# geoeo/ORB_SLAM3_V1.0

Hardware: AMD Instinct MI355X
Metric: frames/sec ORB extract+match, 752x480 8-level 1000-feat; bit-exact kp/desc (higher is better)
Workload: dtype u8

## Files before the change

orb_slam3_v1.0_amd/csrc/fast_common.h:

```cpp
#pragma once
#include <hip/hip_runtime.h>
#include <stdint.h>

namespace orbfe {

constexpr int kFastTW = 64, kFastTH = 32;

constexpr int kFusedPyramidMinFrames = 0;

__device__ __forceinline__ bool arc9(uint32_t m)
{
    uint32_t m2 = m | (m << 16);
    uint32_t r = m2 & (m2 >> 1);
    r &= r >> 2;
    r &= r >> 4;
    r &= m2 >> 8;
    return (r & 0xffffu) != 0;
}

__device__ __forceinline__ bool corner_at_global(const uint8_t* __restrict__ img, int pitch, int x, int y, int th)
{
    const int8_t dy[16] = {3, 3, 2, 1, 0, -1, -2, -3, -3, -3, -2, -1, 0, 1, 2, 3};
    const int8_t dx[16] = {0, 1, 2, 3, 3, 3, 2, 1, 0, -1, -2, -3, -3, -3, -2, -1};
    const int v = img[(size_t)y * pitch + x];
    uint32_t mb = 0, md = 0;
#pragma unroll
    for (int k = 0; k < 16; k++) {
        const int d = (int)img[(size_t)(y + dy[k]) * pitch + x + dx[k]] - v;
        mb |= (uint32_t)(d > th) << k;
        md |= (uint32_t)(d < -th) << k;
    }
    return arc9(mb) || arc9(md);
}

}
```

orb_slam3_v1.0_amd/csrc/kernels_pyramid.hip:

```cpp
#include <algorithm>
#include <cstdlib>

#include "launch.h"

namespace orbfe {

constexpr int kRsTW = 128, kRsTH = 16;
constexpr int kRsMaxRows = 40, kRsMaxCols = 304;

template <int KPASS>
__global__ __launch_bounds__(256) void resize_kernel(const uint8_t* __restrict__ src, size_t srcFrameStride,
                                                     int sw, int sh, int spitch, int srcAligned4,
                                                     uint8_t* __restrict__ dst, size_t dstFrameStride,
                                                     int dw, int dh, int dpitch,
                                                     const uint32_t* __restrict__ xtab,
                                                     const uint32_t* __restrict__ ytab)
{
    __shared__ __attribute__((aligned(16))) uint8_t sSrc[kRsMaxRows][kRsMaxCols];

    const int f = blockIdx.x;
    const int tx0 = blockIdx.y * kRsTW;
    const int ty0 = blockIdx.z * kRsTH;
    const int tid = threadIdx.x;
    const uint8_t* s = src + (size_t)f * srcFrameStride;

    const int x0 = tx0 + (tid & 31) * 4;
    const int yA = ty0 + (tid >> 5), yB = yA + 8;
    const bool colOk = x0 < dw;
    uint4 xt4 = make_uint4(0, 0, 0, 0);
    uint32_t ytA = 0, ytB = 0;
    if (colOk) xt4 = *reinterpret_cast<const uint4*>(xtab + x0);
    if (yA < dh) ytA = ytab[yA];
    if (yB < dh) ytB = ytab[yB];

    const int txLast = min(tx0 + kRsTW, dw) - 1;
    const int tyLast = min(ty0 + kRsTH, dh) - 1;
    const int sx0 = (int)(xtab[tx0] & 0xffffu) & ~3;
    const int sx1 = min((int)(xtab[txLast] & 0xffffu) + 1, sw - 1);
    const int sy0 = (int)(ytab[ty0] & 0xffffu);
    const int sy1 = min((int)(ytab[tyLast] & 0xffffu) + 1, sh - 1);
    const int nrows = sy1 - sy0 + 1;
    const int ndw = (sx1 - sx0) / 4 + 1;
    const bool staged = nrows <= 4 * KPASS && ndw * 4 <= kRsMaxCols;

    if (staged) {
        const int c4l = tid & 63, rl = tid >> 6;
        if (srcAligned4 && ndw <= 64) {
            constexpr int kPass = KPASS;
            const bool cok = c4l < ndw;
            uint32_t off = __umul24((unsigned)(sy0 + rl), (unsigned)spitch) + (unsigned)(sx0 + 4 * c4l);
            const uint32_t step = 4u * (unsigned)spitch;
            uint32_t wv[kPass];
#pragma unroll
            for (int k = 0; k < kPass; k++) {
// ... 42 lines not shown
                const int x2 = min(x1 + 1, sw - 1);
                const uint32_t a = fetch(y1, x1), b = fetch(y1, x2), c = fetch(y2, x1), e = fetch(y2, x2);
                const uint32_t top = __umul24(a, wxc) + __umul24(b, wx);
                const uint32_t bot = __umul24(c, wxc) + __umul24(e, wx);
                const uint32_t v = __umul24(top, wyc) + __umul24(bot, wy) + (1u << 21);
                outw |= (v >> 22) << (8 * i);
            }
            uint8_t* d = dst + (size_t)f * dstFrameStride + __umul24((unsigned)y, (unsigned)dpitch);
            if (nvalid == 4) {
                *reinterpret_cast<uint32_t*>(d + x0) = outw;
            } else {
                for (int i = 0; i < nvalid; i++) d[x0 + i] = (uint8_t)(outw >> (8 * i));
            }
        }
    };
    if (staged)
        body([&](int yy, int xx) -> uint32_t {
            return (&sSrc[0][0])[__umul24((uint32_t)(yy - sy0), (uint32_t)kRsMaxCols) + (uint32_t)(xx - sx0)];
        });
    else
        body([&](int yy, int xx) -> uint32_t { return s[(size_t)yy * spitch + xx]; });
}


constexpr int kPyrWaves = 4;

constexpr int kPyrRows = 7;
constexpr int kPyrSegDw = 96;
constexpr int kPyrStride = 128;


__device__ __forceinline__ uint32_t mad24_vsv(uint32_t a, uint32_t w, uint32_t c)
{
    uint32_t r;
    asm("v_mad_u32_u24 %0, %1, %2, %3" : "=v"(r) : "v"(a), "s"(w), "v"(c));
    return r;
}

__device__ __forceinline__ void pyr_hpass(uint32_t d0, uint32_t d1, uint32_t d2, const uint32_t (&sel)[4], const uint32_t (&wp)[4],
                                          uint32_t (&h)[4])
{
    typedef unsigned short us2 __attribute__((ext_vector_type(2)));
    const uint32_t e0 = __builtin_amdgcn_alignbyte(d1, d0, 3), e1 = __builtin_amdgcn_alignbyte(d2, d1, 3);
#pragma unroll
    for (int i = 0; i < 4; i++) {
        const uint32_t pair = i < 3 ? __builtin_amdgcn_perm(d1, d0, sel[i]) : __builtin_amdgcn_perm(e1, e0, sel[i]);
        h[i] = __builtin_amdgcn_udot2(__builtin_bit_cast(us2, pair), __builtin_bit_cast(us2, wp[i]), 0u, false);
    }
}

__global__ __launch_bounds__(kPyrWaves * 64) void pyramid_kernel(const PipelineDesc* __restrict__ P, int l, int R,
                                                                 const uint8_t* __restrict__ gray0, size_t gray0FrameStride,
                                                                 int gray0Pitch, uint8_t* __restrict__ ws,
                                                                 const uint32_t* __restrict__ tabs)
{
    __shared__ uint32_t sRows[kPyrWaves][kPyrRows][kPyrStride];

    const int f = blockIdx.x;
    const int lane = threadIdx.x & 63;
    const int wave = __builtin_amdgcn_readfirstlane((int)(threadIdx.x >> 6));
    uint32_t* const ring = &sRows[wave][0][0];

    {
        const LevelDesc& S = P->lv[l - 1];
        const LevelDesc& D = P->lv[l];
        const int sw = S.w, sh = S.h, dw = D.w, dh = D.h, dpitch = D.pitch;
        const uint8_t* src = l == 1 ? gray0 + (size_t)f * gray0FrameStride : ws + S.imgOff + (size_t)f * S.imgFrameStride;
        const int spitch = l == 1 ? gray0Pitch : S.pitch;
        uint8_t* dst = ws + D.imgOff + (size_t)f * D.imgFrameStride;
        const uint32_t* xtab = tabs + D.xtabOff;
        const uint32_t* ytab = tabs + D.ytabOff;
        const int strips = (dh + R - 1) / R, chunks = (dw + 255) / 256;
        const __amdgpu_buffer_rsrc_t srsrc =
            __builtin_amdgcn_make_buffer_rsrc(const_cast<uint8_t*>(src), 0, (sh - 1) * spitch + ((sw + 3) & ~3), 0x00020000);
        const __amdgpu_buffer_rsrc_t drsrc = __builtin_amdgcn_make_buffer_rsrc(dst, 0, dh * dpitch, 0x00020000);

        const int task = (int)blockIdx.y * kPyrWaves + wave;
        if (task < strips * chunks) {
            const int strip = task / chunks, chunk = task - strip * chunks;
            const int x0 = chunk * 256 + lane * 4;
            const bool colOk = x0 < dw;
            const int xg = min(x0, (dw - 1) & ~3);
            const uint4 xt4 = *reinterpret_cast<const uint4*>(xtab + xg);
            const uint32_t xt[4] = {xt4.x, xt4.y, xt4.z, xt4.w};
            const uint32_t start = (xt[0] & 0xffffu) & ~3u;
            const uint32_t segBase = (xtab[chunk * 256] & 0xffffu) & ~3u;
            const uint32_t winOff = start - segBase;
            uint32_t sel[4], wp[4];
#pragma unroll
            for (int i = 0; i < 4; i++) {
                const uint32_t o = (xt[i] & 0xffffu) - start - (i == 3 ? 3u : 0u);
                sel[i] = 0x0c000c00u | o | ((o + 1u) << 16);
                const uint32_t wx = xt[i] >> 16;
                wp[i] = (2048u - wx) | (wx << 16);
            }
            const int nvalid = min(4, dw - x0);
            constexpr uint32_t kNowhere = 0x7ffffff0u;
            const uint32_t rowEnd = (uint32_t)((sw + 3) & ~3);
            const uint32_t colA = segBase + 4u * (uint32_t)lane;
            const uint32_t ldA = colA + 4u <= rowEnd ? colA : kNowhere;
            const uint32_t ldB = (lane < kPyrSegDw - 64 && colA + 260u <= rowEnd) ? colA + 256u : kNowhere;
            const uint32_t stX = colOk ? (uint32_t)x0 : kNowhere;
            const bool partial = (dw & 3) != 0;

            const int ys = strip * R, ye = min(ys + R, dh);
            const uint32_t roMax = (uint32_t)((sh - 1) * spitch);
            uint32_t kRound = 1u << 23;
            asm("" : "+v"(kRound));
            uint32_t ytN[4];
            uint32_t ga[kPyrRows], gb[kPyrRows];
            auto request = [&](int yb) {
// ... 48 lines not shown
                                    __builtin_amdgcn_raw_buffer_store_b8((uint8_t)(outw >> (8 * i)), drsrc, (uint32_t)(x0 + i), stRow, 0);
                            }
                        }
                    }
                    stRow += (uint32_t)dpitch;
                }
            }
        }
    }
}

void launch_resize(hipStream_t s, int frames, const uint8_t* src, size_t srcFrameStride, int sw, int sh,
                   int spitch, int srcAligned4, uint8_t* dst, size_t dstFrameStride, int dw, int dh, int dpitch,
                   const uint32_t* xtab, const uint32_t* ytab)
{
    dim3 block(256);
    dim3 grid(frames, (dw + kRsTW - 1) / kRsTW, (dh + kRsTH - 1) / kRsTH);
    const int maxRows = (int)(((long long)(kRsTH - 1) * sh + dh - 1) / dh) + 2;
    if (maxRows <= 24)
        hipLaunchKernelGGL(resize_kernel<6>, grid, block, 0, s, src, srcFrameStride, sw, sh, spitch, srcAligned4, dst,
                           dstFrameStride, dw, dh, dpitch, xtab, ytab);
    else
        hipLaunchKernelGGL(resize_kernel<kRsMaxRows / 4>, grid, block, 0, s, src, srcFrameStride, sw, sh, spitch, srcAligned4,
                           dst, dstFrameStride, dw, dh, dpitch, xtab, ytab);
}


bool pyramid_level_fits(const uint32_t* xtab, const uint32_t* ytab, int sw, int sh, int dw, int dh)
{
    for (int y = 0; y < dh; y++) {
        if ((int)(ytab[y] & 0xffffu) + 1 > sh - 1) return false;
        const int yl = std::min(y + 3, dh - 1);
        if ((int)(ytab[yl] & 0xffffu) + 1 - (int)(ytab[y] & 0xffffu) + 1 > kPyrRows) return false;
    }
    for (int c0 = 0; c0 < dw; c0 += 256) {
        const uint32_t segBase = (xtab[c0] & 0xffffu) & ~3u;
        const int xl = (std::min(c0 + 256, dw) - 1) & ~3;
        const uint32_t startL = (xtab[xl] & 0xffffu) & ~3u;
        if (startL + 12 - segBase > 4u * kPyrSegDw) return false;
    }
    for (int x0 = 0; x0 < dw; x0 += 4) {
        const uint32_t start = (xtab[x0] & 0xffffu) & ~3u;
        for (int i = 0; i < 4 && x0 + i < dw; i++) {
            const uint32_t x1 = xtab[x0 + i] & 0xffffu;
            if ((int)x1 + 1 > sw - 1 || x1 < start) return false;
            const uint32_t o = x1 - start;
            if (i < 3 ? o + 1 > 7 : (o < 3 || o - 3 + 1 > 7)) return false;
        }
    }
    return true;
}

void launch_pyramid_level(hipStream_t s, int frames, const PipelineDesc* dP, int level, int dw, int dh, const uint8_t* gray0,
                          size_t gray0FrameStride, int gray0Pitch, uint8_t* ws, const uint32_t* tabs)
{
#ifdef ORBFE_DIAG
    static const int envR = getenv("ORBFE_PYR_ROWS") ? atoi(getenv("ORBFE_PYR_ROWS")) : 0;
#else
    constexpr int envR = 0;
#endif
    const int R = envR > 0 ? (envR + 3) & ~3 : frames >= 128 ? 8 : 4;
    const int tasks = ((dh + R - 1) / R) * ((dw + 255) / 256);
    hipLaunchKernelGGL(pyramid_kernel, dim3(frames, (tasks + kPyrWaves - 1) / kPyrWaves), dim3(kPyrWaves * 64), 0, s, dP, level, R, gray0,
                       gray0FrameStride, gray0Pitch, ws, tabs);
}


namespace {

struct ChainCtx {
    const uint8_t* src0;
    int pitch0, w0, h0;
    const uint32_t* xtab[3];
    const uint32_t* ytab[3];
    int w[3], h[3];
};

template <int K>
__device__ __forceinline__ uint32_t chain_px(const ChainCtx& c, int x, int y)
{
    const uint32_t xt = c.xtab[K - 1][x], yt = c.ytab[K - 1][y];
    const int sw = K == 1 ? c.w0 : c.w[K - 2], sh = K == 1 ? c.h0 : c.h[K - 2];
    const int x1 = (int)(xt & 0xffffu), y1 = (int)(yt & 0xffffu);
    const uint32_t wx = xt >> 16, wy = yt >> 16;
    const uint32_t wxc = 2048u - wx, wyc = 2048u - wy;
    const int x2 = min(x1 + 1, sw - 1), y2 = min(y1 + 1, sh - 1);
    uint32_t a, b, cc, e;
    if constexpr (K == 1) {
        const uint8_t* r1 = c.src0 + (size_t)y1 * c.pitch0;
        const uint8_t* r2 = c.src0 + (size_t)y2 * c.pitch0;
        a = r1[x1]; b = r1[x2]; cc = r2[x1]; e = r2[x2];
    } else {
        a = chain_px<K - 1>(c, x1, y1); b = chain_px<K - 1>(c, x2, y1);
        cc = chain_px<K - 1>(c, x1, y2); e = chain_px<K - 1>(c, x2, y2);
    }
    const uint32_t top = __umul24(a, wxc) + __umul24(b, wx);
    const uint32_t bot = __umul24(cc, wxc) + __umul24(e, wx);
    const uint32_t v = __umul24(top, wyc) + __umul24(bot, wy) + (1u << 21);
    return v >> 22;
}

__global__ __launch_bounds__(256) void pyramid_chain_kernel(const PipelineDesc* __restrict__ P, int l0, int depth,
                                                            const uint8_t* __restrict__ gray0, size_t gray0FrameStride, int gray0Pitch,
                                                            uint8_t* __restrict__ ws, const uint32_t* __restrict__ tabs,
                                                            uint32_t* __restrict__ zero, int nZeroPerFrame)
{
    const int f = blockIdx.y;
    if (zero && blockIdx.x == 0)
        for (int i = threadIdx.x; i < nZeroPerFrame; i += 256) zero[(size_t)f * nZeroPerFrame + i] = 0;
    ChainCtx c;
    const LevelDesc& S = P->lv[l0];
    c.src0 = l0 == 0 ? gray0 + (size_t)f * gray0FrameStride : ws + S.imgOff + (size_t)f * S.imgFrameStride;
    c.pitch0 = l0 == 0 ? gray0Pitch : S.pitch;
    c.w0 = S.w;
    c.h0 = S.h;
    int np[3] = {0, 0, 0};
#pragma unroll
    for (int k = 0; k < 3; k++) {
// ... 36 lines not shown
```

orb_slam3_v1.0_amd/csrc/launch.h:

```cpp
#pragma once
#include "orbfe_internal.h"

namespace orbfe {

void launch_resize(hipStream_t s, int frames, const uint8_t* src, size_t srcFrameStride, int sw, int sh,
                   int spitch, int srcAligned4, uint8_t* dst, size_t dstFrameStride, int dw, int dh, int dpitch,
                   const uint32_t* xtab, const uint32_t* ytab);

bool pyramid_level_fits(const uint32_t* xtab, const uint32_t* ytab, int sw, int sh, int dw, int dh);
void launch_pyramid_level(hipStream_t s, int frames, const PipelineDesc* dP, int level, int dw, int dh, const uint8_t* gray0,
                          size_t gray0FrameStride, int gray0Pitch, uint8_t* ws, const uint32_t* tabs);

void launch_pyramid_chain(hipStream_t s, int frames, const PipelineDesc* dP, const PipelineDesc& hostP, int l0, int depth,
                          const uint8_t* gray0, size_t gray0FrameStride, int gray0Pitch, uint8_t* ws, const uint32_t* tabs,
                          uint32_t* zero = nullptr, int nZeroPerFrame = 0);

void fast_tiles_for(int w, int h, int* tx, int* ty);
uint32_t fast_tile_info(int level, int tileX, int tileY);
void launch_fast_blur(hipStream_t s, int frames, int tileBase, int nTiles, bool buildNext, const PipelineDesc* dP,
                      const uint32_t* dTileInfo, const uint32_t* dTabs, const uint8_t* gray0, size_t gray0FrameStride, int gray0Pitch,
                      int gray0Aligned4, uint8_t* ws, uint32_t* cand, uint32_t* counters, uint16_t* tileRows);
bool fast_next_level_fits(const uint32_t* xtab, const uint32_t* ytab, int sw, int sh, int dw, int dh, uint32_t* own);

int quadtree_node_capacity(int maxNodeCap);
size_t quadtree_scratch_bytes_per_block(int maxNodeCap);
void launch_quadtree(hipStream_t s, int frames, int nLevels, int maxNodeCap, const PipelineDesc* dP,
                     const uint32_t* cand, uint16_t* nodeOf, uint32_t* counters, uint32_t* lvlKp,
                     const uint8_t* gray0, size_t gray0FrameStride, int gray0Pitch, const uint8_t* ws,
                     const uint16_t* tileRows, uint8_t* scratch);

void launch_orient_brief(hipStream_t s, int frames, int kpCapFrame, const PipelineDesc* dP, const uint8_t* gray0,
                         size_t gray0FrameStride, int gray0Pitch, const uint8_t* ws, const uint32_t* counters,
                         const uint32_t* lvlKp, orbfe_keypoint* kpOut, uint8_t* descOut, int* nOut,
                         int* perLevelOut, int* statusOut, const int* kpBase, int nLevels);

void launch_clock_probe(hipStream_t s, unsigned long long* dOut2, unsigned ticks);

}
```

orb_slam3_v1.0_amd/csrc/orbfe_host.cpp:

```cpp
#include <atomic>
#include <cmath>
#include <cstdio>
#include <cstdlib>
#include <cstring>
#include <map>
#include <mutex>
#include <new>
#include <condition_variable>
#include <functional>
#include <string>
#include <thread>
#include <vector>

#include "launch.h"
#include "fast_common.h"
#include "match.h"
#include "match_common.h"
#include "match_proj.h"
#include "keyframe.h"
#include "marginalize.h"
#include "poseimu_math.h"
#include "prep.h"
#include "vocab.h"

// ... 18 lines not shown
        Key key;
        hipGraphExec_t exec;
    };
    std::vector<Entry> entries;
    hipGraphExec_t find(const Key& key) const
    {
        for (const Entry& e : entries)
            if (memcmp(&e.key, &key, sizeof key) == 0) return e.exec;
        return nullptr;
    }
    void insert(const Key& key, hipGraphExec_t exec, size_t bound)
    {
        if (entries.size() >= bound) drop();
        entries.push_back({key, exec});
    }
    void drop()
    {
        for (Entry& e : entries)
            if (e.exec) (void)hipGraphExecDestroy(e.exec);
        entries.clear();
    }
};

}

struct orbfe_map;
struct orbfe_stream;

struct orbfe_handle {
    orbfe_params prm{};
    int device = 0;
    int nLevels = 0;
    double scaleFactorD = 0.0;
    float sf[kMaxLevels]{}, inv[kMaxLevels]{}, sig2[kMaxLevels]{}, invSig2[kMaxLevels]{};
    PipelineDesc P{};
    PipelineDesc* dP = nullptr;
    int maxBatch = 1;
    int maxNodeCap = 0;

    uint8_t* ws = nullptr;
    size_t wsBytes = 0;
    uint32_t* dCand = nullptr;
    uint16_t* dNodeOf = nullptr;
    size_t candWordsPerBatch = 0;
    uint32_t* dCounters = nullptr;
    uint32_t* dLvlKp = nullptr;
    uint16_t* dTileRows = nullptr;
    uint8_t* dQtScratch = nullptr;
    uint32_t* dTabs = nullptr;
    uint32_t* dTileInfo = nullptr;
    bool pyrFits[kMaxLevels]{};
    bool fusedFits[kMaxLevels]{};
    int fusedMinFrames = kFusedPyramidMinFrames;
    bool fusedSplitOnly = false;
    float* dSf = nullptr;

    uint8_t* dIn = nullptr;
    int dInPitch = 0;
    uint8_t* hIn = nullptr;
    uint8_t* dOutBlock = nullptr;
    uint8_t* hOutBlock = nullptr;
    size_t outBlockBytes = 0, offStatus = 0, offPer = 0, offKp = 0, offDesc = 0;
    orbfe_keypoint* dKp = nullptr;
    uint8_t* dDesc = nullptr;
    int* dN = nullptr;
    int* dStatus = nullptr;
    int* dPer = nullptr;
    orbfe_keypoint* hKp = nullptr;
    uint8_t* hDesc = nullptr;
    int* hN = nullptr;
    int* hStatus = nullptr;
    int* hPer = nullptr;
    std::map<int, hipGraphExec_t> graphs;
    bool useGraph = true;
    int graphCaptures = 0, captureFailures = 0;
    int captureFailStreak = 0;

    hipStream_t stream = nullptr;
    bool timing = false;
    hipEvent_t ev[kEventSets][ORBFE_NUM_STAGES]{};
    int evHead = 0, evCount = 0;

    const uint8_t* lastGray = nullptr;
    size_t lastStride = 0;
    int lastPitch = 0, lastBatch = 0;

    MatchScratch match;

    struct TrackKey {
        int Mb, inPitch, gridCols, gridRows, farPoints;
        float minX, minY, invW, invH, th, nnRatio, thFar;
        const void* map;
    };
    MatchScratch trackMatch;
    ChainBlocks trk;
    int trkCapM = 0;
    GraphCache<TrackKey> trackGraphs;
    struct RefKey {
        int inPitch, levelsup, checkOri;
        float nnRatio;
        unsigned long long vocabSerial;
    };
    ChainBlocks ref;
    int refCapFlags = 0;
    GraphCache<RefKey> refGraphs;
    struct IniKey {
// ... 243 lines not shown
    PipelineDesc& P = h->P;
    memset(&P, 0, sizeof P);
    P.nLevels = nL;
    P.nFast = p->n_fast_features;
    P.iniTh = p->ini_th_fast;
    P.minTh = p->min_th_fast;
    size_t wsOff = 0, candOff = 0, tabOff = 0;
    int tileBase = 0, kpBase = 0;
    const size_t B = (size_t)p->max_batch;
    int status = ORBFE_OK;
    for (int l = 0; l < nL; l++) {
        LevelDesc& L = P.lv[l];
        if (l == 0) {
            L.w = p->image_width;
            L.h = p->image_height;
        } else {
            L.w = cv_round_f(h->inv[l] * (float)p->image_width);
            L.h = cv_round_f(h->inv[l] * (float)p->image_height);
        }
        if (L.w < 16 || L.h < 16) { status = ORBFE_ERR_UNSUPPORTED; break; }
        L.pitch = (int)align_up((size_t)L.w, kPitchAlign);
        L.nFeatures = fpl[l];
        L.nIni = (int)roundf((float)L.w / (float)L.h);
        if (L.nIni < 1) { status = ORBFE_ERR_UNSUPPORTED; break; }
        L.hX = (float)L.w / (float)L.nIni;
        L.nodeCap = std::max(L.nFeatures + 3, 4 * L.nIni);
        L.candCap = ((L.w + 1) / 2) * ((L.h + 1) / 2);
        fast_tiles_for(L.w, L.h, &L.tilesX, &L.tilesY);
        L.tileBase = tileBase;
        tileBase += L.tilesX * L.tilesY;
        L.kpBase = kpBase;
        kpBase += L.nodeCap;
        L.invScale = h->inv[l];
        L.scaledPatch = (int)(kPatch * h->inv[l]);
        const size_t frameBytes = align_up((size_t)L.pitch * L.h, 256);
        L.imgFrameStride = frameBytes;
        L.blurFrameStride = frameBytes;
        if (l > 0) {
            L.imgOff = wsOff;
            wsOff += frameBytes * B;
        }
        L.blurOff = wsOff;
        wsOff += frameBytes * B;
        L.candOff = candOff;
        candOff += (size_t)L.candCap * B;
        tabOff = align_up(tabOff, 4);
        L.xtabOff = tabOff;
        tabOff += align_up((size_t)L.w, 4);
        L.ytabOff = tabOff;
        tabOff += align_up((size_t)L.h, 4);
        tabOff = align_up(tabOff, 4);
        L.ownOff = (uint32_t)tabOff;
        tabOff += (size_t)L.tilesX + L.tilesY + 2;
        h->maxNodeCap = std::max(h->maxNodeCap, L.nodeCap);
    }
    if (status == ORBFE_OK && quadtree_node_capacity(h->maxNodeCap) == 0) status = ORBFE_ERR_UNSUPPORTED;
    if (status != ORBFE_OK) {
        delete h;
        return status;
    }
    P.kpCapFrame = kpBase;
    P.totalTiles = tileBase;
    for (int l = 0; l < 8; l++) P.tileBaseTab[l] = l < nL ? P.lv[l].tileBase : 0x7fffffff;
    h->wsBytes = wsOff;
    h->candWordsPerBatch = candOff;

    std::vector<uint32_t> tabs(tabOff ? tabOff : 1, 0);
    for (int l = 1; l < nL; l++) {
        fill_resize_table(tabs, P.lv[l].xtabOff, P.lv[l - 1].w, P.lv[l].w);
        fill_resize_table(tabs, P.lv[l].ytabOff, P.lv[l - 1].h, P.lv[l].h);
    }

    for (int l = 1; l < nL; l++)
        if (pyramid_level_fits(tabs.data() + P.lv[l].xtabOff, tabs.data() + P.lv[l].ytabOff, P.lv[l - 1].w, P.lv[l - 1].h, P.lv[l].w,
                               P.lv[l].h))
            h->pyrFits[l] = true;
    for (int l = 1; l < nL; l++)
        h->fusedFits[l] = fast_next_level_fits(tabs.data() + P.lv[l].xtabOff, tabs.data() + P.lv[l].ytabOff, P.lv[l - 1].w, P.lv[l - 1].h,
                                               P.lv[l].w, P.lv[l].h, tabs.data() + P.lv[l - 1].ownOff) && h->pyrFits[l];

#define CREATE_CHK(call)                                                  \
    do {                                                                  \
        hipError_t e_ = (call);                                           \
        if (e_ != hipSuccess) {                                           \
            int rc_ = e_ == hipErrorOutOfMemory ? ORBFE_ERR_OUT_OF_MEMORY : ORBFE_ERR_HIP; \
            destroy_impl(h);                                              \
            return rc_;                                                   \
        }                                                                 \
    } while (0)

    CREATE_CHK(hipStreamCreateWithFlags(&h->stream, hipStreamNonBlocking));
    CREATE_CHK(hipMalloc(&h->dP, sizeof(PipelineDesc)));
    CREATE_CHK(hipMalloc(&h->ws, h->wsBytes + 256));
    CREATE_CHK(hipMalloc(&h->dCand, candOff * sizeof(uint32_t)));
    CREATE_CHK(hipMalloc(&h->dNodeOf, candOff * sizeof(uint16_t)));
    CREATE_CHK(hipMalloc(&h->dCounters, B * nL * kCntWords * sizeof(uint32_t)));
    CREATE_CHK(hipMalloc(&h->dLvlKp, B * (size_t)P.kpCapFrame * sizeof(uint32_t)));
    CREATE_CHK(hipMalloc(&h->dTileRows, B * (size_t)P.totalTiles * 32 * sizeof(uint16_t)));
    if (quadtree_scratch_bytes_per_block(h->maxNodeCap))
        CREATE_CHK(hipMalloc(&h->dQtScratch, quadtree_scratch_bytes_per_block(h->maxNodeCap) * B * nL));
    CREATE_CHK(hipMalloc(&h->dTabs, tabs.size() * sizeof(uint32_t)));
    {
        std::vector<uint32_t> info((size_t)P.totalTiles);
        for (int l = 0; l < nL; l++)
            for (int ty = 0; ty < P.lv[l].tilesY; ty++)
                for (int tx = 0; tx < P.lv[l].tilesX; tx++) info[P.lv[l].tileBase + ty * P.lv[l].tilesX + tx] = fast_tile_info(l, tx, ty);
        CREATE_CHK(hipMalloc(&h->dTileInfo, info.size() * sizeof(uint32_t)));
        CREATE_CHK(copy_sync(h->dTileInfo, info.data(), info.size() * sizeof(uint32_t), hipMemcpyHostToDevice, h->stream));
    }
    CREATE_CHK(hipMalloc(&h->dSf, kMaxLevels * sizeof(float)));
    CREATE_CHK(copy_sync(h->dSf, h->sf, kMaxLevels * sizeof(float), hipMemcpyHostToDevice, h->stream));
    CREATE_CHK(copy_sync(h->dP, &P, sizeof P, hipMemcpyHostToDevice, h->stream));
    CREATE_CHK(copy_sync(h->dTabs, tabs.data(), tabs.size() * sizeof(uint32_t), hipMemcpyHostToDevice, h->stream));

    h->dInPitch = (int)align_up((size_t)p->image_width, kPitchAlign);
    const size_t inFrame = (size_t)h->dInPitch * p->image_height;
    const size_t cap = (size_t)P.kpCapFrame;
    CREATE_CHK(hipMalloc(&h->dIn, inFrame * B));
    CREATE_CHK(hipHostMalloc(&h->hIn, inFrame * B));
    {
        size_t off = 0;
        auto take = [&](size_t bytes) { const size_t o = off; off = align_up(off + bytes, 256); return o; };
        take(B * sizeof(int));
        h->offStatus = take(B * sizeof(int));
        h->offPer = take(B * nL * sizeof(int));
        h->offKp = take(B * cap * sizeof(orbfe_keypoint));
        h->offDesc = take(B * cap * ORBFE_DESC_BYTES);
        h->outBlockBytes = off;
    }
    CREATE_CHK(hipMalloc(&h->dOutBlock, h->outBlockBytes));
    CREATE_CHK(hipHostMalloc(&h->hOutBlock, h->outBlockBytes));
    h->dN = reinterpret_cast<int*>(h->dOutBlock);
    h->dStatus = reinterpret_cast<int*>(h->dOutBlock + h->offStatus);
    h->dPer = reinterpret_cast<int*>(h->dOutBlock + h->offPer);
    h->dKp = reinterpret_cast<orbfe_keypoint*>(h->dOutBlock + h->offKp);
    h->dDesc = h->dOutBlock + h->offDesc;
    h->hN = reinterpret_cast<int*>(h->hOutBlock);
    h->hStatus = reinterpret_cast<int*>(h->hOutBlock + h->offStatus);
    h->hPer = reinterpret_cast<int*>(h->hOutBlock + h->offPer);
    h->hKp = reinterpret_cast<orbfe_keypoint*>(h->hOutBlock + h->offKp);
    h->hDesc = h->hOutBlock + h->offDesc;
#ifdef ORBFE_DIAG
    h->useGraph = getenv("ORBFE_NO_GRAPH") == nullptr;
    if (const char* e = getenv("ORBFE_FUSED_PYRAMID")) {
        h->fusedMinFrames = atoi(e) ? 1 : 0;
        h->fusedSplitOnly = atoi(e) == 2;
    }
#endif
    CREATE_CHK(hipEventCreateWithFlags(&h->evExtract, hipEventDisableTiming));
    CREATE_CHK(hipEventCreateWithFlags(&h->evMatch, hipEventDisableTiming));
    h->match.busy = h->evMatch;
    for (auto& set : h->ev)
        for (auto& e : set) CREATE_CHK(hipEventCreate(&e));
#undef CREATE_CHK
    *out = h;
    return ORBFE_OK;
}

void orbfe_destroy(orbfe_handle* h) { destroy_impl(h); }

int orbfe_get_levels(const orbfe_handle* h) { return h ? h->nLevels : 0; }
float orbfe_get_scale_factor(const orbfe_handle* h) { return h ? (float)h->scaleFactorD : 0.f; }

int orbfe_get_scale_tables(const orbfe_handle* h, float* sf, float* inv, float* s2, float* is2)
{
    if (!h) return ORBFE_ERR_INVALID_ARG;
    for (int i = 0; i < h->nLevels; i++) {
        if (sf) sf[i] = h->sf[i];
        if (inv) inv[i] = h->inv[i];
        if (s2) s2[i] = h->sig2[i];
        if (is2) is2[i] = h->invSig2[i];
    }
    return ORBFE_OK;
}

int orbfe_get_level_info(const orbfe_handle* h, int* fpl, int* lw, int* lh)
{
    if (!h) return ORBFE_ERR_INVALID_ARG;
    for (int i = 0; i < h->nLevels; i++) {
        if (fpl) fpl[i] = h->P.lv[i].nFeatures;
        if (lw) lw[i] = h->P.lv[i].w;
        if (lh) lh[i] = h->P.lv[i].h;
    }
    return ORBFE_OK;
}

int orbfe_max_keypoints(const orbfe_handle* h) { return h ? h->P.kpCapFrame : 0; }

int orbfe_set_stage_timing(orbfe_handle* h, int enabled)
{
    if (!h) return ORBFE_ERR_INVALID_ARG;
    h->timing = enabled != 0;
    h->evHead = h->evCount = 0;
    return ORBFE_OK;
}

int orbfe_get_stage_ms(orbfe_handle* h, float ms[ORBFE_NUM_STAGES], int* n_calls)
{
    if (!h || !ms || !n_calls) return ORBFE_ERR_INVALID_ARG;
    HIPCHK(h, hipSetDevice(h->device));
// ... 7 lines not shown
            HIPCHK(h, hipEventElapsedTime(&t, e[s], e[s + 1]));
            ms[s] += t;
        }
        float t = 0.f;
        HIPCHK(h, hipEventElapsedTime(&t, e[0], e[ORBFE_NUM_STAGES - 1]));
        ms[ORBFE_NUM_STAGES - 1] += t;
    }
    *n_calls = n;
    return ORBFE_OK;
}

static int extract_chain(orbfe_handle* h, const uint8_t* d_gray, size_t frame_stride, int pitch, int batch,
                         orbfe_keypoint* d_kp, uint8_t* d_desc, int* d_n, int* d_per, int* d_status, void* stream_);

int orbfe_extract_batch_device(orbfe_handle* h, const uint8_t* d_gray, size_t frame_stride, int pitch,
                               int batch, orbfe_keypoint* d_kp, uint8_t* d_desc, int* d_n, int* d_per,
                               void* stream_)
{
    if (!h) return ORBFE_ERR_INVALID_ARG;
    std::lock_guard<std::mutex> lk(h->mu);
    return extract_chain(h, d_gray, frame_stride, pitch, batch, d_kp, d_desc, d_n, d_per, nullptr, stream_);
}

}

static int extract_chain(orbfe_handle* h, const uint8_t* d_gray, size_t frame_stride, int pitch, int batch,
                         orbfe_keypoint* d_kp, uint8_t* d_desc, int* d_n, int* d_per, int* d_status, void* stream_)
{
    if (!h || !d_gray || !d_kp || !d_desc || !d_n) return ORBFE_ERR_INVALID_ARG;
    if (batch < 1 || batch > h->maxBatch || pitch < h->prm.image_width || pitch >= (1 << 24)) return ORBFE_ERR_INVALID_ARG;
    const int aligned4 = ((reinterpret_cast<uintptr_t>(d_gray) | (uintptr_t)pitch | (uintptr_t)frame_stride) & 3u) == 0;
    const size_t rowEnd = aligned4 ? (size_t)((h->prm.image_width + 3) & ~3) : (size_t)h->prm.image_width;
    if (batch > 1 && frame_stride < (size_t)pitch * (h->prm.image_height - 1) + rowEnd) return ORBFE_ERR_INVALID_ARG;
    if ((size_t)pitch * (h->prm.image_height - 1) + (size_t)((h->prm.image_width + 3) & ~3) >= (size_t)0x7ffffff0u)
        return ORBFE_ERR_INVALID_ARG;
    HIPCHK(h, hipSetDevice(h->device));
    hipStream_t s = stream_ ? (hipStream_t)stream_ : h->stream;
    hipStreamCaptureStatus capturing = hipStreamCaptureStatusNone;
    if (hipStreamIsCapturing(s, &capturing) != hipSuccess) (void)hipGetLastError();
    if (capturing == hipStreamCaptureStatusNone) {
        const int rc = scratch_acquire(h, h->extractUsed, h->extractStream, h->evExtract, s);
        if (rc != ORBFE_OK) return rc;
    }
    const PipelineDesc& P = h->P;
    const int nL = P.nLevels;
    hipEvent_t* ev = nullptr;
    if (h->timing) {
        ev = h->ev[h->evHead];
        h->evHead = (h->evHead + 1) % kEventSets;
        h->evCount++;
    }
    const bool fused = h->fusedMinFrames > 0 && batch >= h->fusedMinFrames && nL > 1;
    const bool chainPyr = !fused && (long long)batch * nL <= 64 && !ev && nL > 1;
    if (!chainPyr) HIPCHK(h, hipMemsetAsync(h->dCounters, 0, (size_t)batch * nL * kCntWords * sizeof(uint32_t), s));
    if (ev) HIPCHK(h, hipEventRecord(ev[0], s));
    for (int l = 1; chainPyr && l < nL;) {
        const int left = nL - l;
        const int depth = left >= 5 ? 2 : std::min(left, 3);
        launch_pyramid_chain(s, batch, h->dP, P, l - 1, depth, d_gray, frame_stride, pitch, h->ws, h->dTabs,
                             l == 1 ? h->dCounters : nullptr, nL * kCntWords);
        l += depth;
    }
    auto pyramid_level = [&](int l) {
        const LevelDesc& S = P.lv[l - 1];
        const LevelDesc& D = P.lv[l];
        if (h->pyrFits[l] && (l > 1 || aligned4)) {
            launch_pyramid_level(s, batch, h->dP, l, D.w, D.h, d_gray, frame_stride, pitch, h->ws, h->dTabs);
            return;
        }
        const uint8_t* src = l == 1 ? d_gray : h->ws + S.imgOff;
        const size_t sstride = l == 1 ? frame_stride : S.imgFrameStride;
        const int spitch = l == 1 ? pitch : S.pitch;
        launch_resize(s, batch, src, sstride, S.w, S.h, spitch, l == 1 ? aligned4 : 1, h->ws + D.imgOff, D.imgFrameStride, D.w, D.h,
                      D.pitch, h->dTabs + D.xtabOff, h->dTabs + D.ytabOff);
    };
    for (int l = chainPyr || (fused && !h->fusedSplitOnly) ? nL : 1; l < nL; l++) pyramid_level(l);
    if (ev) HIPCHK(h, hipEventRecord(ev[1], s));
    if (fused) {
        for (int l = 0; l < nL; l++) {
            const bool build = l + 1 < nL && h->fusedFits[l + 1] && !h->fusedSplitOnly;
            launch_fast_blur(s, batch, P.lv[l].tileBase, P.lv[l].tilesX * P.lv[l].tilesY, build, h->dP, h->dTileInfo, h->dTabs, d_gray,
                             frame_stride, pitch, aligned4, h->ws, h->dCand, h->dCounters, h->dTileRows);
            if (l + 1 < nL && !build && !h->fusedSplitOnly) pyramid_level(l + 1);
        }
    } else {
        launch_fast_blur(s, batch, 0, P.totalTiles, false, h->dP, h->dTileInfo, h->dTabs, d_gray, frame_stride, pitch, aligned4, h->ws,
                         h->dCand, h->dCounters, h->dTileRows);
    }
    if (ev) HIPCHK(h, hipEventRecord(ev[2], s));
    launch_quadtree(s, batch, nL, h->maxNodeCap, h->dP, h->dCand, h->dNodeOf, h->dCounters, h->dLvlKp, d_gray, frame_stride,
                    pitch, h->ws, h->dTileRows, h->dQtScratch);
    if (ev) HIPCHK(h, hipEventRecord(ev[3], s));
    int kpBase[kMaxLevels];
    for (int l = 0; l < nL; l++) kpBase[l] = P.lv[l].kpBase;
    launch_orient_brief(s, batch, P.kpCapFrame, h->dP, d_gray, frame_stride, pitch, h->ws, h->dCounters, h->dLvlKp,
                        d_kp, d_desc, d_n, d_per, d_status, kpBase, nL);
    if (ev) HIPCHK(h, hipEventRecord(ev[4], s));
    HIPCHK(h, hipGetLastError());
    h->lastGray = d_gray;
    h->lastStride = frame_stride;
    h->lastPitch = pitch;
    h->lastBatch = batch;
    if (capturing == hipStreamCaptureStatusNone) return extract_scratch_release(h, s);
    return ORBFE_OK;
}

extern "C" {

static int check_device_flags(orbfe_handle* h, int batch)
{
    for (int b = 0; b < batch; b++)
        if (h->hStatus[b]) {
            char buf[128];
            snprintf(buf, sizeof buf, "device guard flags 0x%x at frame %d", (unsigned)h->hStatus[b], b);
            h->err = buf;
            return ORBFE_ERR_INTERNAL;
        }
    return ORBFE_OK;
}

static int extract_host_enqueue(orbfe_handle* h, int batch, int inPitch, hipStream_t s)
{
    const int nL = h->nLevels;
    const size_t inFrame = (size_t)h->dInPitch * h->prm.image_height;
    const size_t cap = (size_t)h->P.kpCapFrame;
    const int rc = extract_chain(h, h->dIn, inFrame, inPitch, batch, h->dKp, h->dDesc, h->dN, h->dPer, h->dStatus, s);
    if (rc != ORBFE_OK) return rc;
    if (batch == h->maxBatch) {
        HIPCHK(h, hipMemcpyAsync(h->hOutBlock, h->dOutBlock, h->outBlockBytes, hipMemcpyDeviceToHost, s));
// ... 2657 lines not shown
```

Measured before the change: 228,200.

## Add paired pyramid kernel and fold counter clearing into first pyramid launch

Adds a kernel that builds two consecutive pyramid levels in one pass. Each wave keeps the intermediate level rows in an LDS ring buffer and resizes them again for the next level, which saves one launch and one global re-read per pair. A host-side check works out column and row ownership tables so every intermediate row is stored exactly once. Separately, the counter hipMemsetAsync is replaced by zeroing done inside the first pyramid launch. The pair path is gated by kPyramidPairMinFrames, which is 0, so by default it stays off unless ORBFE_PYR_PAIR is set in diag builds. The memset folding does run by default on the non-chain, non-fused path.

```diff
diff --git a/orb_slam3_v1.0_amd/csrc/fast_common.h b/orb_slam3_v1.0_amd/csrc/fast_common.h
--- a/orb_slam3_v1.0_amd/csrc/fast_common.h
+++ b/orb_slam3_v1.0_amd/csrc/fast_common.h
@@ -7,6 +7,8 @@
 constexpr int kFastTW = 64, kFastTH = 32;
 
 constexpr int kFusedPyramidMinFrames = 0;
+
+constexpr int kPyramidPairMinFrames = 0;
 
 __device__ __forceinline__ bool arc9(uint32_t m)
 {
diff --git a/orb_slam3_v1.0_amd/csrc/kernels_pyramid.hip b/orb_slam3_v1.0_amd/csrc/kernels_pyramid.hip
--- a/orb_slam3_v1.0_amd/csrc/kernels_pyramid.hip
+++ b/orb_slam3_v1.0_amd/csrc/kernels_pyramid.hip
@@ -1,5 +1,6 @@
 #include <algorithm>
 #include <cstdlib>
+#include <vector>
 
 #include "launch.h"
 
@@ -148,11 +149,14 @@
 __global__ __launch_bounds__(kPyrWaves * 64) void pyramid_kernel(const PipelineDesc* __restrict__ P, int l, int R,
                                                                  const uint8_t* __restrict__ gray0, size_t gray0FrameStride,
                                                                  int gray0Pitch, uint8_t* __restrict__ ws,
-                                                                 const uint32_t* __restrict__ tabs)
+                                                                 const uint32_t* __restrict__ tabs, uint32_t* __restrict__ zero,
+                                                                 int nZeroPerFrame)
 {
     __shared__ uint32_t sRows[kPyrWaves][kPyrRows][kPyrStride];
 
     const int f = blockIdx.x;
+    if (zero && blockIdx.y == 0)
+        for (int i = threadIdx.x; i < nZeroPerFrame; i += kPyrWaves * 64) zero[(size_t)f * nZeroPerFrame + i] = 0;
     const int lane = threadIdx.x & 63;
     const int wave = __builtin_amdgcn_readfirstlane((int)(threadIdx.x >> 6));
     uint32_t* const ring = &sRows[wave][0][0];
@@ -307,7 +311,7 @@
 }
 
 void launch_pyramid_level(hipStream_t s, int frames, const PipelineDesc* dP, int level, int dw, int dh, const uint8_t* gray0,
-                          size_t gray0FrameStride, int gray0Pitch, uint8_t* ws, const uint32_t* tabs)
+                          size_t gray0FrameStride, int gray0Pitch, uint8_t* ws, const uint32_t* tabs, uint32_t* zero, int nZeroPerFrame)
 {
 #ifdef ORBFE_DIAG
     static const int envR = getenv("ORBFE_PYR_ROWS") ? atoi(getenv("ORBFE_PYR_ROWS")) : 0;
@@ -317,8 +321,279 @@
     const int R = envR > 0 ? (envR + 3) & ~3 : frames >= 128 ? 8 : 4;
     const int tasks = ((dh + R - 1) / R) * ((dw + 255) / 256);
     hipLaunchKernelGGL(pyramid_kernel, dim3(frames, (tasks + kPyrWaves - 1) / kPyrWaves), dim3(kPyrWaves * 64), 0, s, dP, level, R, gray0,
-                       gray0FrameStride, gray0Pitch, ws, tabs);
-}
+                       gray0FrameStride, gray0Pitch, ws, tabs, zero, nZeroPerFrame);
+}
+
+
+constexpr int kPairWaves = 3;
+constexpr int kPairRows = 16;
+constexpr int kPairRing = 8;
+constexpr int kPairMinCw = 64;
+constexpr int kPairWaveDw = kPairRing * 64 + kPyrRows * kPyrSegDw;
+
+__global__ __launch_bounds__(kPairWaves * 64) void pyramid_pair_kernel(const PipelineDesc* __restrict__ P, int l, int cw, uint32_t pairTab,
+                                                                      const uint8_t* __restrict__ gray0, size_t gray0FrameStride,
+                                                                      int gray0Pitch, uint8_t* __restrict__ ws,
+                                                                      const uint32_t* __restrict__ tabs, uint32_t* __restrict__ zero,
+                                                                      int nZeroPerFrame)
+{
+    __shared__ uint32_t sMem[kPairWaves][kPairWaveDw];
+
+    const int f = blockIdx.x;
+    if (zero && blockIdx.y == 0)
+        for (int i = threadIdx.x; i < nZeroPerFrame; i += kPairWaves * 64) zero[(size_t)f * nZeroPerFrame + i] = 0;
+    const int lane = threadIdx.x & 63;
+    const int wave = __builtin_amdgcn_readfirstlane((int)(threadIdx.x >> 6));
+    uint32_t* const ring = &sMem[wave][0];
+    uint32_t* const stage = ring + kPairRing * 64;
+
+    const LevelDesc& A = P->lv[l - 1];
+    const LevelDesc& B = P->lv[l];
+    const LevelDesc& C = P->lv[l + 1];
+    const int wA = A.w, hA = A.h, wB = B.w, hB = B.h, pitchB = B.pitch, wC = C.w, hC = C.h, pitchC = C.pitch;
+    const uint8_t* src = l == 1 ? gray0 + (size_t)f * gray0FrameStride : ws + A.imgOff + (size_t)f * A.imgFrameStride;
+    const int spitch = l == 1 ? gray0Pitch : A.pitch;
+    uint8_t* dstB = ws + B.imgOff + (size_t)f * B.imgFrameStride;
+    uint8_t* dstC = ws + C.imgOff + (size_t)f * C.imgFrameStride;
+    const uint32_t* xtB = tabs + B.xtabOff;
+    const uint32_t* ytB = tabs + B.ytabOff;
+    const uint32_t* xtC = tabs + C.xtabOff;
+    const uint32_t* ytC = tabs + C.ytabOff;
+    const int strips = (hC + kPairRows - 1) / kPairRows, chunks = (wC + cw - 1) / cw;
+    const uint32_t* colOwn = tabs + pairTab;
+    const uint32_t* rowOwn = colOwn + chunks + 1;
+    const __amdgpu_buffer_rsrc_t srsrc =
+        __builtin_amdgcn_make_buffer_rsrc(const_cast<uint8_t*>(src), 0, (hA - 1) * spitch + ((wA + 3) & ~3), 0x00020000);
+    const __amdgpu_buffer_rsrc_t rsrcB = __builtin_amdgcn_make_buffer_rsrc(dstB, 0, hB * pitchB, 0x00020000);
+    const __amdgpu_buffer_rsrc_t rsrcC = __builtin_amdgcn_make_buffer_rsrc(dstC, 0, hC * pitchC, 0x00020000);
+
+    const int task = (int)blockIdx.y * kPairWaves + wave;
+    if (task >= strips * chunks) return;
+    const int strip = task / chunks, chunk = task - strip * chunks;
+    const int bLo = (int)colOwn[chunk], ownHiX = (int)colOwn[chunk + 1];
+    const int ownLoY = (int)rowOwn[strip], ownHiY = (int)rowOwn[strip + 1];
+    constexpr uint32_t kNowhere = 0x7ffffff0u;
+
+    const int xB0 = bLo + lane * 4;
+    uint32_t selB[4], wpB[4], winOffA;
+    const uint32_t segBase = (xtB[bLo] & 0xffffu) & ~3u;
+    {
+        const uint4 xt4 = *reinterpret_cast<const uint4*>(xtB + min(xB0, (wB - 1) & ~3));
+        const uint32_t xt[4] = {xt4.x, xt4.y, xt4.z, xt4.w};
+        const uint32_t start = (xt[0] & 0xffffu) & ~3u;
+        winOffA = min(start - segBase, 4u * (kPyrSegDw - 3));
+#pragma unroll
+        for (int i = 0; i < 4; i++) {
+            const uint32_t o = (xt[i] & 0xffffu) - start - (i == 3 ? 3u : 0u);
+            selB[i] = 0x0c000c00u | o | ((o + 1u) << 16);
+            const uint32_t wx = xt[i] >> 16;
+            wpB[i] = (2048u - wx) | (wx << 16);
+        }
+    }
+    const bool ownB = xB0 < ownHiX;
+    const int nvalidB = min(4, wB - xB0);
+    const uint32_t stXB = ownB ? (uint32_t)xB0 : kNowhere;
+    const bool partialB = (wB & 3) != 0;
+    const uint32_t rowEnd = (uint32_t)((wA + 3) & ~3);
+    const uint32_t colA = segBase + 4u * (uint32_t)lane;
+    const uint32_t ldA = colA + 4u <= rowEnd ? colA : kNowhere;
+    const uint32_t ldB = (lane < kPyrSegDw - 64 && colA + 260u <= rowEnd) ? colA + 256u : kNowhere;
+
+    const int xC0 = chunk * cw + lane * 4;
+    const bool colOkC = lane * 4 < cw && xC0 < wC;
+    uint32_t selC[4], wpC[4], winOffC;
+    {
+        const uint4 xt4 = *reinterpret_cast<const uint4*>(xtC + min(xC0, (wC - 1) & ~3));
+        const uint32_t xt[4] = {xt4.x, xt4.y, xt4.z, xt4.w};
+        const uint32_t start = (xt[0] & 0xffffu) & ~3u;
+        winOffC = min(start - (uint32_t)bLo, 252u);
+#pragma unroll
+        for (int i = 0; i < 4; i++) {
+            const uint32_t o = (xt[i] & 0xffffu) - start - (i == 3 ? 3u : 0u);
+            selC[i] = 0x0c000c00u | o | ((o + 1u) << 16);
+            const uint32_t wx = xt[i] >> 16;
+            wpC[i] = (2048u - wx) | (wx << 16);
+        }
+    }
+    const int nvalidC = min(4, wC - xC0);
+    const uint32_t stXC = colOkC ? (uint32_t)xC0 : kNowhere;
+    const bool partialC = (wC & 3) != 0;
+
+    const int ys = strip * kPairRows, ye = min(ys + kPairRows, hC);
+    const int bStart = ownLoY;
+    const int bEnd = strip == strips - 1 ? hB : (int)(ytC[ye - 1] & 0xffffu) + 2;
+    const uint32_t roMax = (uint32_t)((hA - 1) * spitch);
+    uint32_t kRound = 1u << 23;
+    asm("" : "+v"(kRound));
+
+    auto blend = [&](const uint32_t* wt, const uint32_t* wb, const uint32_t (&sel)[4], const uint32_t (&wp)[4], uint32_t ytEntry) {
+        uint32_t hT[4], hU[4];
+        pyr_hpass(wt[0], wt[1], wt[2], sel, wp, hT);
+        pyr_hpass(wb[0], wb[1], wb[2], sel, wp, hU);
+        const uint32_t wy4 = (ytEntry >> 16) * 4u, wyc4 = 8192u - wy4;
+        uint32_t v[4];
+#pragma unroll
+        for (int i = 0; i < 4; i++) v[i] = mad24_vsv(hU[i], wy4, mad24_vsv(hT[i], wyc4, kRound));
+        const uint32_t lo = __builtin_amdgcn_perm(v[1], v[0], 0x0c0c0703u);
+        const uint32_t hi = __builtin_amdgcn_perm(v[3], v[2], 0x0c0c0703u);
+        return lo | (hi << 16);
+    };
+    auto put = [&](uint32_t outw, const __amdgpu_buffer_rsrc_t& rsrc, bool partial, bool colOk, int nvalid, int x0, uint32_t stX,
+                   uint32_t stRow) {
+        if (!partial) {
+            __builtin_amdgcn_raw_buffer_store_b32(outw, rsrc, stX, stRow, 0);
+        } else if (colOk) {
+            if (nvalid >= 4) {
+                __builtin_amdgcn_raw_buffer_store_b32(outw, rsrc, (uint32_t)x0, stRow, 0);
+            } else {
+                for (int i = 0; i < nvalid; i++)
+                    __builtin_amdgcn_raw_buffer_store_b8((uint8_t)(outw >> (8 * i)), rsrc, (uint32_t)(x0 + i), stRow, 0);
+            }
+        }
+    };
+
+    uint32_t ytN[4];
+    uint32_t ga[kPyrRows], gb[kPyrRows];
+    auto request = [&](int b) {
+#pragma unroll
+        for (int k = 0; k < 4; k++) ytN[k] = ytB[min(b + k, hB - 1)];
+        uint32_t ro = (ytN[0] & 0xffffu) * (uint32_t)spitch;
+#pragma unroll
+        for (int j = 0; j < kPyrRows; j++) {
+            const uint32_t roc = min(ro, roMax);
+            ga[j] = __builtin_amdgcn_raw_buffer_load_b32(srsrc, ldA, roc, 0);
+            gb[j] = __builtin_amdgcn_raw_buffer_load_b32(srsrc, ldB, roc, 0);
+            ro += (uint32_t)spitch;
+        }
+    };
+    request(bStart);
+    int yC = ys;
+    uint32_t ytC4[4];
+#pragma unroll
+    for (int k = 0; k < 4; k++) ytC4[k] = ytC[min(yC + k, hC - 1)];
+    uint32_t stRowC = (uint32_t)(ys * pitchC);
+    uint32_t stRowB = (uint32_t)(bStart * pitchB);
+#pragma unroll 1
+    for (int b = bStart; b < bEnd; b += 4) {
+        uint32_t yt[4];
+#pragma unroll
+        for (int k = 0; k < 4; k++) yt[k] = ytN[k];
+        const int rA = (int)(yt[0] & 0xffffu);
+#pragma unroll
+        for (int j = 0; j < kPyrRows; j++) stage[j * kPyrSegDw + lane] = ga[j];
+        if (lane < kPyrSegDw - 64) {
+#pragma unroll
+            for (int j = 0; j < kPyrRows; j++) stage[j * kPyrSegDw + 64 + lane] = gb[j];
+        }
+        if (b + 4 < bEnd) request(b + 4);
+#pragma unroll
+        for (int k = 0; k < 4; k++) {
+            if (b + k >= bEnd) break;
+            const int jt = (int)(yt[k] & 0xffffu) - rA;
+            const uint32_t* wt = reinterpret_cast<const uint32_t*>(reinterpret_cast<const uint8_t*>(stage + jt * kPyrSegDw) + winOffA);
+            const uint32_t outw = blend(wt, wt + kPyrSegDw, selB, wpB, yt[k]);
+            ring[((b + k) & (kPairRing - 1)) * 64 + lane] = outw;
+            if (b + k < ownHiY) put(outw, rsrcB, partialB, ownB, nvalidB, xB0, stXB, stRowB);
+            stRowB += (uint32_t)pitchB;
+        }
+        const int bDone = b + 4;
+        uint32_t ytU[4];
+        bool go[4];
+        int n = 0;
+#pragma unroll
+        for (int k = 0; k < 4; k++) {
+            ytU[k] = ytC4[k];
+            go[k] = yC + k < ye && (int)(ytU[k] & 0xffffu) + 1 < bDone;
+            n += go[k] ? 1 : 0;
+        }
+        yC += n;
+#pragma unroll
+        for (int k = 0; k < 4; k++) ytC4[k] = ytC[min(yC + k, hC - 1)];
+#pragma unroll
+        for (int k = 0; k < 4; k++) {
+            if (go[k]) {
+                const int y1 = (int)(ytU[k] & 0xffffu);
+                const uint32_t* wt = reinterpret_cast<const uint32_t*>(
+                    reinterpret_cast<const uint8_t*>(ring + (y1 & (kPairRing - 1)) * 64) + winOffC);
+                const uint32_t* wb = reinterpret_cast<const uint32_t*>(
+                    reinterpret_cast<const uint8_t*>(ring + ((y1 + 1) & (kPairRing - 1)) * 64) + winOffC);
+                const uint32_t outw = blend(wt, wb, selC, wpC, ytU[k]);
+                put(outw, rsrcC, partialC, colOkC, nvalidC, xC0, stXC, stRowC);
+                stRowC += (uint32_t)pitchC;
+            }
+        }
+    }
+}
+
+int pyramid_pair_fits(const uint32_t* xtB, const uint32_t* ytB, const uint32_t* xtC, const uint32_t* ytC, int wB, int hB, int wC, int hC,
+                      uint32_t* own, int ownCap)
+{
+    auto near = [](const uint32_t* t, int i) { return (int)(t[i] & 0xffffu); };
+    const int strips = (hC + kPairRows - 1) / kPairRows;
+    int cw = 0, chunks = 0;
+    const int nMin = (wC + 255) / 256;
+    for (int n = nMin; cw == 0; n++) {
+        const int w = ((wC + n - 1) / n + 3) & ~3;
+        if (n > nMin && w < kPairMinCw) return 0;
+        const int nc = (wC + w - 1) / w;
+        if (nc + 1 + strips + 1 > ownCap) return 0;
+        bool ok = true;
+        for (int c = 0; c <= nc; c++) own[c] = c == nc ? (uint32_t)wB : (uint32_t)(near(xtC, c * w) & ~3);
+        for (int c = 0; c < nc && ok; c++) {
+            const int bLo = (int)own[c], hi = (int)own[c + 1];
+            const int xLast = std::min((c + 1) * w, wC) - 1;
+            const int need = std::max(hi - 1, near(xtC, xLast) + 1);
+            ok = hi > bLo && bLo < wB && need < wB && need - bLo < 256;
+            for (int x0 = c * w; x0 <= xLast && ok; x0 += 4) ok = (near(xtC, x0) & ~3) - bLo <= 252;
+            if (ok) ok = (near(xtB, need & ~3) & ~3) + 12 - (near(xtB, bLo) & ~3) <= 4 * kPyrSegDw;
+        }
+        if (ok) { cw = w; chunks = nc; }
+    }
+    uint32_t* rowOwn = own + chunks + 1;
+    for (int s = 0; s <= strips; s++) rowOwn[s] = s == strips ? (uint32_t)hB : s == 0 ? 0u : (uint32_t)near(ytC, s * kPairRows);
+    std::vector<int> stored((size_t)hB, 0);
+    for (int s = 0; s < strips; s++) {
+        const int ys = s * kPairRows, ye = std::min(ys + kPairRows, hC);
+        const int bStart = (int)rowOwn[s], ownHi = (int)rowOwn[s + 1];
+        const int bEnd = s == strips - 1 ? hB : near(ytC, ye - 1) + 2;
+        if (ownHi <= bStart || ownHi > bEnd || bEnd > hB) return 0;
+        int slot[kPairRing];
+        for (int& v : slot) v = -1;
+        int yC = ys;
+        for (int b = bStart; b < bEnd; b += 4) {
+            const int r0 = near(ytB, b);
+            for (int k = 0; k < 4 && b + k < bEnd; k++) {
+                if (near(ytB, b + k) + 1 - r0 + 1 > kPyrRows) return 0;
+                slot[(b + k) & (kPairRing - 1)] = b + k;
+                if (b + k < ownHi) stored[b + k]++;
+            }
+            int n = 0;
+            for (int k = 0; k < 4; k++) {
+                if (yC + k >= ye || near(ytC, yC + k) + 1 >= b + 4) continue;
+                const int y1 = near(ytC, yC + k);
+                if (n != k || slot[y1 & (kPairRing - 1)] != y1 || slot[(y1 + 1) & (kPairRing - 1)] != y1 + 1) return 0;
+                n++;
+            }
+            yC += n;
+        }
+        if (yC != ye) return 0;
+    }
+    for (int y = 0; y < hB; y++)
+        if (stored[y] != 1) return 0;
+    return cw;
+}
+
+void launch_pyramid_pair(hipStream_t s, int frames, const PipelineDesc* dP, const PipelineDesc& hostP, int level, int cw, uint32_t pairTab,
+                         const uint8_t* gray0, size_t gray0FrameStride, int gray0Pitch, uint8_t* ws, const uint32_t* tabs, uint32_t* zero,
+                         int nZeroPerFrame)
+{
+    const LevelDesc& C = hostP.lv[level + 1];
+    const int tasks = ((C.h + kPairRows - 1) / kPairRows) * ((C.w + cw - 1) / cw);
+    hipLaunchKernelGGL(pyramid_pair_kernel, dim3(frames, (tasks + kPairWaves - 1) / kPairWaves), dim3(kPairWaves * 64), 0, s, dP, level, cw,
+                       pairTab, gray0, gray0FrameStride, gray0Pitch, ws, tabs, zero, nZeroPerFrame);
+}
+
+int pyramid_pair_table_words(int wC, int hC) { return wC / kPairMinCw + 3 + (hC + kPairRows - 1) / kPairRows + 1; }
 
 
 namespace {
diff --git a/orb_slam3_v1.0_amd/csrc/launch.h b/orb_slam3_v1.0_amd/csrc/launch.h
--- a/orb_slam3_v1.0_amd/csrc/launch.h
+++ b/orb_slam3_v1.0_amd/csrc/launch.h
@@ -9,7 +9,15 @@
 
 bool pyramid_level_fits(const uint32_t* xtab, const uint32_t* ytab, int sw, int sh, int dw, int dh);
 void launch_pyramid_level(hipStream_t s, int frames, const PipelineDesc* dP, int level, int dw, int dh, const uint8_t* gray0,
-                          size_t gray0FrameStride, int gray0Pitch, uint8_t* ws, const uint32_t* tabs);
+                          size_t gray0FrameStride, int gray0Pitch, uint8_t* ws, const uint32_t* tabs,
+                          uint32_t* zero = nullptr, int nZeroPerFrame = 0);
+
+int pyramid_pair_table_words(int wC, int hC);
+int pyramid_pair_fits(const uint32_t* xtB, const uint32_t* ytB, const uint32_t* xtC, const uint32_t* ytC, int wB, int hB, int wC, int hC,
+                      uint32_t* own, int ownCap);
+void launch_pyramid_pair(hipStream_t s, int frames, const PipelineDesc* dP, const PipelineDesc& hostP, int level, int cw, uint32_t pairTab,
+                         const uint8_t* gray0, size_t gray0FrameStride, int gray0Pitch, uint8_t* ws, const uint32_t* tabs,
+                         uint32_t* zero = nullptr, int nZeroPerFrame = 0);
 
 void launch_pyramid_chain(hipStream_t s, int frames, const PipelineDesc* dP, const PipelineDesc& hostP, int l0, int depth,
                           const uint8_t* gray0, size_t gray0FrameStride, int gray0Pitch, uint8_t* ws, const uint32_t* tabs,
diff --git a/orb_slam3_v1.0_amd/csrc/orbfe_host.cpp b/orb_slam3_v1.0_amd/csrc/orbfe_host.cpp
--- a/orb_slam3_v1.0_amd/csrc/orbfe_host.cpp
+++ b/orb_slam3_v1.0_amd/csrc/orbfe_host.cpp
@@ -94,6 +94,9 @@
     bool pyrFits[kMaxLevels]{};
     bool fusedFits[kMaxLevels]{};
     int fusedMinFrames = kFusedPyramidMinFrames;
+    int pyrPairFits[kMaxLevels]{};
+    uint32_t pyrPairTab[kMaxLevels]{};
+    int pairMinFrames = kPyramidPairMinFrames;
     bool fusedSplitOnly = false;
     float* dSf = nullptr;
 
@@ -443,6 +446,10 @@
         tabOff = align_up(tabOff, 4);
         L.ownOff = (uint32_t)tabOff;
         tabOff += (size_t)L.tilesX + L.tilesY + 2;
+        if (l >= 2) {
+            h->pyrPairTab[l - 1] = (uint32_t)tabOff;
+            tabOff += (size_t)pyramid_pair_table_words(L.w, L.h);
+        }
         h->maxNodeCap = std::max(h->maxNodeCap, L.nodeCap);
     }
     if (status == ORBFE_OK && quadtree_node_capacity(h->maxNodeCap) == 0) status = ORBFE_ERR_UNSUPPORTED;
@@ -469,6 +476,12 @@
     for (int l = 1; l < nL; l++)
         h->fusedFits[l] = fast_next_level_fits(tabs.data() + P.lv[l].xtabOff, tabs.data() + P.lv[l].ytabOff, P.lv[l - 1].w, P.lv[l - 1].h,
                                                P.lv[l].w, P.lv[l].h, tabs.data() + P.lv[l - 1].ownOff) && h->pyrFits[l];
+
+    for (int l = 1; l + 1 < nL; l++)
+        if (h->pyrFits[l] && h->pyrFits[l + 1])
+            h->pyrPairFits[l] = pyramid_pair_fits(tabs.data() + P.lv[l].xtabOff, tabs.data() + P.lv[l].ytabOff, tabs.data() + P.lv[l + 1].xtabOff,
+                                                  tabs.data() + P.lv[l + 1].ytabOff, P.lv[l].w, P.lv[l].h, P.lv[l + 1].w, P.lv[l + 1].h,
+                                                  tabs.data() + h->pyrPairTab[l], pyramid_pair_table_words(P.lv[l + 1].w, P.lv[l + 1].h));
 
 #define CREATE_CHK(call)                                                  \
     do {                                                                  \
@@ -537,6 +550,7 @@
         h->fusedMinFrames = atoi(e) ? 1 : 0;
         h->fusedSplitOnly = atoi(e) == 2;
     }
+    if (const char* e = getenv("ORBFE_PYR_PAIR")) h->pairMinFrames = atoi(e) ? 1 : 0;
 #endif
     CREATE_CHK(hipEventCreateWithFlags(&h->evExtract, hipEventDisableTiming));
     CREATE_CHK(hipEventCreateWithFlags(&h->evMatch, hipEventDisableTiming));
@@ -650,7 +664,8 @@
     }
     const bool fused = h->fusedMinFrames > 0 && batch >= h->fusedMinFrames && nL > 1;
     const bool chainPyr = !fused && (long long)batch * nL <= 64 && !ev && nL > 1;
-    if (!chainPyr) HIPCHK(h, hipMemsetAsync(h->dCounters, 0, (size_t)batch * nL * kCntWords * sizeof(uint32_t), s));
+    const bool pyrClears = !chainPyr && !fused && nL > 1 && h->pyrFits[1] && aligned4;
+    if (!chainPyr && !pyrClears) HIPCHK(h, hipMemsetAsync(h->dCounters, 0, (size_t)batch * nL * kCntWords * sizeof(uint32_t), s));
     if (ev) HIPCHK(h, hipEventRecord(ev[0], s));
     for (int l = 1; chainPyr && l < nL;) {
         const int left = nL - l;
@@ -663,7 +678,8 @@
         const LevelDesc& S = P.lv[l - 1];
         const LevelDesc& D = P.lv[l];
         if (h->pyrFits[l] && (l > 1 || aligned4)) {
-            launch_pyramid_level(s, batch, h->dP, l, D.w, D.h, d_gray, frame_stride, pitch, h->ws, h->dTabs);
+            launch_pyramid_level(s, batch, h->dP, l, D.w, D.h, d_gray, frame_stride, pitch, h->ws, h->dTabs,
+                                 l == 1 && pyrClears ? h->dCounters : nullptr, nL * kCntWords);
             return;
         }
         const uint8_t* src = l == 1 ? d_gray : h->ws + S.imgOff;
@@ -672,7 +688,16 @@
         launch_resize(s, batch, src, sstride, S.w, S.h, spitch, l == 1 ? aligned4 : 1, h->ws + D.imgOff, D.imgFrameStride, D.w, D.h,
                       D.pitch, h->dTabs + D.xtabOff, h->dTabs + D.ytabOff);
     };
-    for (int l = chainPyr || (fused && !h->fusedSplitOnly) ? nL : 1; l < nL; l++) pyramid_level(l);
+    const bool pairs = h->pairMinFrames > 0 && batch >= h->pairMinFrames;
+    for (int l = chainPyr || (fused && !h->fusedSplitOnly) ? nL : 1; l < nL;) {
+        if (pairs && l + 1 < nL && h->pyrPairFits[l] && (l > 1 || aligned4)) {
+            launch_pyramid_pair(s, batch, h->dP, P, l, h->pyrPairFits[l], h->pyrPairTab[l], d_gray, frame_stride, pitch, h->ws, h->dTabs,
+                                l == 1 && pyrClears ? h->dCounters : nullptr, nL * kCntWords);
+            l += 2;
+        } else {
+            pyramid_level(l++);
+        }
+    }
     if (ev) HIPCHK(h, hipEventRecord(ev[1], s));
     if (fused) {
         for (int l = 0; l < nL; l++) {
```

Result: no change. 228,600, median of 3 (+0.2%).
